# khuongnd6/ViT_torch

Hardware: AMD Instinct MI355X
Metric: images/sec fwd+bwd ViT-B/16 224^2 bs=256/GPU (higher is better)
Workload: dtype bf16; 1 GPU; dino_vitb16 224x224 fwd+CE+bwd+SGD(momentum) step, batch 256/GPU, 10 classes, random-init weights; global_batch=256, residual_stream=bf16, parallelism=dp1, hip_graph=True

## Files before the change

### vit_torch_amd/csrc/layernorm.hip

```cpp
#include <atomic>
#include <initializer_list>
#include <type_traits>
#include "common.h"

namespace {

constexpr int LN_MAXV = 8;

template <int NV, typename TX, typename TY>
__global__ __launch_bounds__(256) void ln_fwd_kernel(const TX* __restrict__ x, int64_t xs,
                                                     const float* __restrict__ gamma,
                                                     const float* __restrict__ beta,
                                                     TY* __restrict__ y, int64_t ys,
                                                     float* __restrict__ mean_out,
                                                     float* __restrict__ rstd_out,
                                                     int64_t M, int D, float eps) {
  const int lane = threadIdx.x & 63, w = threadIdx.x >> 6;
  for (int64_t row = (int64_t)blockIdx.x * 4 + w; row < M; row += (int64_t)gridDim.x * 4) {
  const TX* xr = x + row * xs;
  f32x4 v[NV];
  float s = 0.f;
#pragma unroll
  for (int i = 0; i < NV; ++i) v[i] = load4<TX>(xr + min((i * 64 + lane) * 4, D - 4));
#pragma unroll
  for (int i = 0; i < NV; ++i) {
    const int c = (i * 64 + lane) * 4;
    if (c < D) s += (v[i][0] + v[i][1]) + (v[i][2] + v[i][3]);
  }
  const float mean = wave_sum(s) / (float)D;
  float q = 0.f;
#pragma unroll
  for (int i = 0; i < NV; ++i) {
    const int c = (i * 64 + lane) * 4;
    if (c < D) {
#pragma unroll
      for (int j = 0; j < 4; ++j) { const float d = v[i][j] - mean; q += d * d; }
    }
  }
  const float var = wave_sum(q) / (float)D;
  const float rstd = rsqrtf(var + eps);
  if (lane == 0) {
    if (mean_out) mean_out[row] = mean;
    if (rstd_out) rstd_out[row] = rstd;
  }
  TY* yr = y + row * ys;
#pragma unroll
  for (int i = 0; i < NV; ++i) {
    const int c = (i * 64 + lane) * 4;
    const int cc = min(c, D - 4);
    const f32x4 g = *reinterpret_cast<const f32x4*>(gamma + cc);
    const f32x4 b = *reinterpret_cast<const f32x4*>(beta + cc);
    if (c < D) {
      f32x4 o;
#pragma unroll
      for (int j = 0; j < 4; ++j) o[j] = (v[i][j] - mean) * rstd * g[j] + b[j];
      store4<TY>(yr + c, o);
    }
  }
  }
}

template <int NV, typename TDY, typename TX, typename TG, typename TGB>
__global__ __launch_bounds__(256) void ln_bwd_kernel(const TDY* __restrict__ dy, int64_t dys,
                                                     const TX* __restrict__ x, int64_t xs,
                                                     const float* __restrict__ mean,
                                                     const float* __restrict__ rstd,
                                                     const float* __restrict__ gamma,
                                                     const TG* g_in, TG* g_out, int64_t gstride,
                                                     TGB* __restrict__ gb_out, int64_t gbs,
                                                     float* __restrict__ part, int want_gsum,
                                                     const float* __restrict__ gb_scale,
                                                     const float* __restrict__ gb_rowscale, int64_t rpg,
                                                     int64_t M, int D) {
  extern __shared__ __attribute__((aligned(16))) float red[];
  const int lane = threadIdx.x & 63, w = threadIdx.x >> 6;
  f32x4 gam[NV], dg[NV], db[NV], gs[NV];
#pragma unroll
  for (int i = 0; i < NV; ++i) {
    const int c = (i * 64 + lane) * 4;
    const f32x4 z = {0.f, 0.f, 0.f, 0.f};
    dg[i] = z; db[i] = z; gam[i] = z; gs[i] = z;
    if (c < D) gam[i] = *reinterpret_cast<const f32x4*>(gamma + c);
  }
  const float invD = 1.f / (float)D;
  for (int64_t row = (int64_t)blockIdx.x * 4 + w; row < M; row += (int64_t)gridDim.x * 4) {
    const float mu = mean[row], rs = rstd[row];
    const TDY* dyr = dy + row * dys;
    const TX* xr = x + row * xs;
    f32x4 xh[NV], dv[NV];
    float s1 = 0.f, s2 = 0.f;
#pragma unroll
    for (int i = 0; i < NV; ++i) {
      const int cc = min((i * 64 + lane) * 4, D - 4);
      xh[i] = load4<TX>(xr + cc);
      dv[i] = load4<TDY>(dyr + cc);
    }
#pragma unroll
    for (int i = 0; i < NV; ++i) {
      const int c = (i * 64 + lane) * 4;
      if (c < D) {
        const f32x4 xv = xh[i];
#pragma unroll
        for (int j = 0; j < 4; ++j) {
          xh[i][j] = (xv[j] - mu) * rs;
          dg[i][j] += dv[i][j] * xh[i][j];
          db[i][j] += dv[i][j];
          dv[i][j] *= gam[i][j];
          s1 += dv[i][j];
          s2 += dv[i][j] * xh[i][j];
        }
      }
    }
    const float c1 = wave_sum(s1) * invD, c2 = wave_sum(s2) * invD;
    float rsc = 1.f;
    if (gb_rowscale) rsc = gb_rowscale[(uint32_t)row / (uint32_t)rpg];
    f32x4 gin[NV];
    if (g_in) {
#pragma unroll
      for (int i = 0; i < NV; ++i) gin[i] = load4<TG>(g_in + row * gstride + min((i * 64 + lane) * 4, D - 4));
    }
#pragma unroll
    for (int i = 0; i < NV; ++i) {
      const int c = (i * 64 + lane) * 4;
      if (c < D) {
        f32x4 o;
#pragma unroll
        for (int j = 0; j < 4; ++j) o[j] = rs * (dv[i][j] - c1 - xh[i][j] * c2);
        if (g_in) {
#pragma unroll
          for (int j = 0; j < 4; ++j) o[j] += gin[i][j];
        }
        store4<TG>(g_out + row * gstride + c, o);
        if (gb_scale) {
          const f32x4 sc = *reinterpret_cast<const f32x4*>(gb_scale + c);
#pragma unroll
          for (int j = 0; j < 4; ++j) o[j] *= sc[j];
        }
        if (gb_rowscale) {
#pragma unroll
          for (int j = 0; j < 4; ++j) o[j] *= rsc;
        }
        if (gb_out) store4<TGB>(gb_out + row * gbs + c, o);
#pragma unroll
        for (int j = 0; j < 4; ++j) gs[i][j] += o[j];
      }
    }
  }
  float* prow = part + (int64_t)blockIdx.x * 3 * D;
#pragma unroll 1
  for (int pass = 0; pass < (want_gsum ? 3 : 2); ++pass) {
#pragma unroll
    for (int i = 0; i < NV; ++i) {
      const int c = (i * 64 + lane) * 4;
      if (c < D) *reinterpret_cast<f32x4*>(red + w * D + c) = pass == 0 ? dg[i] : (pass == 1 ? db[i] : gs[i]);
    }
    __syncthreads();
    for (int c = threadIdx.x; c < D; c += 256)
      prow[pass * D + c] = (red[c] + red[D + c]) + (red[2 * D + c] + red[3 * D + c]);
    __syncthreads();
  }
}

template <typename T> __device__ __forceinline__ void load8(const T* p, float (&o)[8]);
template <> __device__ __forceinline__ void load8<float>(const float* p, float (&o)[8]) {
  const f32x4 a = *reinterpret_cast<const f32x4*>(p), b = *reinterpret_cast<const f32x4*>(p + 4);
  o[0] = a[0]; o[1] = a[1]; o[2] = a[2]; o[3] = a[3]; o[4] = b[0]; o[5] = b[1]; o[6] = b[2]; o[7] = b[3];
}
template <> __device__ __forceinline__ void load8<bf16>(const bf16* p, float (&o)[8]) {
  const bf16x8 v = *reinterpret_cast<const bf16x8*>(p);
#pragma unroll
  for (int i = 0; i < 8; ++i) o[i] = (float)v[i];
}
template <typename T> __device__ __forceinline__ void store8(T* p, const float (&v)[8]);
template <> __device__ __forceinline__ void store8<float>(float* p, const float (&v)[8]) {
  *reinterpret_cast<f32x4*>(p) = f32x4{v[0], v[1], v[2], v[3]};
  *reinterpret_cast<f32x4*>(p + 4) = f32x4{v[4], v[5], v[6], v[7]};
}
template <> __device__ __forceinline__ void store8<bf16>(bf16* p, const float (&v)[8]) {
  bf16x8 o;
#pragma unroll
  for (int i = 0; i < 8; ++i) o[i] = (bf16)v[i];
  *reinterpret_cast<bf16x8*>(p) = o;
}
template <int LPR> __device__ __forceinline__ float group_sum(float v) {
#pragma unroll
  for (int o = LPR / 2; o > 0; o >>= 1) v += __shfl_xor(v, o);
  return v;
}

template <int LPR, int NV, typename TX, typename TY>
__global__ __launch_bounds__(256) void ln_fwd8_kernel(const TX* __restrict__ x, int64_t xs, const float* __restrict__ gamma,
                                                      const float* __restrict__ beta, TY* __restrict__ y, int64_t ys,
                                                      float* __restrict__ mean_out, float* __restrict__ rstd_out,
                                                      int64_t M, int D, float eps) {
  constexpr int RPW = 64 / LPR;
  const int lane = threadIdx.x & 63, w = threadIdx.x >> 6;
  const int sub = lane / LPR, l = lane % LPR;
  const int64_t groups = (M + RPW - 1) / RPW;
  const float invD = 1.f / (float)D;
  for (int64_t grp = (int64_t)blockIdx.x * 4 + w; grp < groups; grp += (int64_t)gridDim.x * 4) {
    const int64_t row = grp * RPW + sub;
    const bool live = row < M;
    const TX* xr = x + (live ? row : M - 1) * xs;
    float v[NV][8];
#pragma unroll
    for (int i = 0; i < NV; ++i) load8<TX>(xr + min((i * LPR + l) * 8, D - 8), v[i]);
    float s = 0.f;
#pragma unroll
    for (int i = 0; i < NV; ++i)
      if ((i * LPR + l) * 8 < D) {
#pragma unroll
        for (int j = 0; j < 8; ++j) s += v[i][j];
      }
    const float mean = group_sum<LPR>(s) * invD;
    float q = 0.f;
#pragma unroll
    for (int i = 0; i < NV; ++i)
      if ((i * LPR + l) * 8 < D) {
#pragma unroll
        for (int j = 0; j < 8; ++j) { const float d = v[i][j] - mean; q += d * d; }
      }
    const float rstd = rsqrtf(group_sum<LPR>(q) * invD + eps);
    if (l == 0 && live) {
      if (mean_out) mean_out[row] = mean;
      if (rstd_out) rstd_out[row] = rstd;
    }
    TY* yr = y + row * ys;
#pragma unroll
    for (int i = 0; i < NV; ++i) {
      const int c = (i * LPR + l) * 8;
      float g[8], b[8];
      load8<float>(gamma + min(c, D - 8), g);
      load8<float>(beta + min(c, D - 8), b);
      if (c < D && live) {
        float o[8];
#pragma unroll
        for (int j = 0; j < 8; ++j) o[j] = (v[i][j] - mean) * rstd * g[j] + b[j];
        store8<TY>(yr + c, o);
      }
    }
  }
}

template <int LPR, int NV, typename TDY, typename TX, typename TG, typename TGB>
__global__ __launch_bounds__(256) void ln_bwd8_kernel(const TDY* __restrict__ dy, int64_t dys, const TX* __restrict__ x, int64_t xs,
                                                      const float* __restrict__ mean, const float* __restrict__ rstd,
                                                      const float* __restrict__ gamma, const TG* g_in, TG* g_out, int64_t gstride,
                                                      TGB* __restrict__ gb_out, int64_t gbs, float* __restrict__ part, int want_gsum,
                                                      const float* __restrict__ gb_scale, const float* __restrict__ gb_rowscale,
                                                      int64_t rpg, int64_t M, int D) {
  extern __shared__ __attribute__((aligned(16))) float red[];
  constexpr int RPW = 64 / LPR;
  const int lane = threadIdx.x & 63, w = threadIdx.x >> 6;
  const int sub = lane / LPR, l = lane % LPR;
  float gam[NV][8], dg[NV][8], db[NV][8], gs[NV][8];
#pragma unroll
  for (int i = 0; i < NV; ++i) {
    load8<float>(gamma + min((i * LPR + l) * 8, D - 8), gam[i]);
#pragma unroll
    for (int j = 0; j < 8; ++j) { dg[i][j] = 0.f; db[i][j] = 0.f; gs[i][j] = 0.f; }
  }
  const float invD = 1.f / (float)D;
  const int64_t groups = (M + RPW - 1) / RPW;
  for (int64_t grp = (int64_t)blockIdx.x * 4 + w; grp < groups; grp += (int64_t)gridDim.x * 4) {
    const int64_t row = grp * RPW + sub;
    const bool live = row < M;
    const int64_t r = live ? row : M - 1;
    const float mu = mean[r], rs = rstd[r];
    float xh[NV][8], dv[NV][8], gin[NV][8];
#pragma unroll
    for (int i = 0; i < NV; ++i) {
      const int cc = min((i * LPR + l) * 8, D - 8);
      load8<TX>(x + r * xs + cc, xh[i]);
      load8<TDY>(dy + r * dys + cc, dv[i]);
    }
    if (g_in) {
#pragma unroll
      for (int i = 0; i < NV; ++i) load8<TG>(g_in + r * gstride + min((i * LPR + l) * 8, D - 8), gin[i]);
    }
    float s1 = 0.f, s2 = 0.f;
#pragma unroll
    for (int i = 0; i < NV; ++i)
      if ((i * LPR + l) * 8 < D && live) {
#pragma unroll
        for (int j = 0; j < 8; ++j) {
          xh[i][j] = (xh[i][j] - mu) * rs;
          dg[i][j] += dv[i][j] * xh[i][j];
          db[i][j] += dv[i][j];
          dv[i][j] *= gam[i][j];
          s1 += dv[i][j];
          s2 += dv[i][j] * xh[i][j];
        }
      }
    const float c1 = group_sum<LPR>(s1) * invD, c2 = group_sum<LPR>(s2) * invD;
    float rsc = 1.f;
    if (gb_rowscale) rsc = gb_rowscale[(uint32_t)r / (uint32_t)rpg];
#pragma unroll
    for (int i = 0; i < NV; ++i) {
      const int c = (i * LPR + l) * 8;
      if (c < D && live) {
        float o[8];
#pragma unroll
        for (int j = 0; j < 8; ++j) o[j] = rs * (dv[i][j] - c1 - xh[i][j] * c2);
        if (g_in) {
#pragma unroll
          for (int j = 0; j < 8; ++j) o[j] += gin[i][j];
        }
        store8<TG>(g_out + row * gstride + c, o);
        if (gb_scale) {
          float sc[8];
          load8<float>(gb_scale + c, sc);
#pragma unroll
          for (int j = 0; j < 8; ++j) o[j] *= sc[j];
        }
        if (gb_rowscale) {
#pragma unroll
          for (int j = 0; j < 8; ++j) o[j] *= rsc;
        }
        if (gb_out) store8<TGB>(gb_out + row * gbs + c, o);
#pragma unroll
        for (int j = 0; j < 8; ++j) gs[i][j] += o[j];
      }
    }
  }
  float* prow = part + (int64_t)blockIdx.x * 3 * D;
  const int slot = w * RPW + sub;
#pragma unroll 1
  for (int pass = 0; pass < (want_gsum ? 3 : 2); ++pass) {
#pragma unroll
    for (int i = 0; i < NV; ++i) {
      const int c = (i * LPR + l) * 8;
      float t[8];
#pragma unroll
      for (int j = 0; j < 8; ++j) t[j] = pass == 0 ? dg[i][j] : (pass == 1 ? db[i][j] : gs[i][j]);
      if (c < D) store8<float>(red + slot * D + c, t);
    }
    __syncthreads();
    for (int c = threadIdx.x; c < D; c += 256) {
      float a = 0.f;
#pragma unroll
      for (int t = 0; t < 4 * RPW; ++t) a += red[t * D + c];
      prow[pass * D + c] = a;
    }
    __syncthreads();
  }
}

template <int LPR, int NV, typename T>
__global__ __launch_bounds__(256) void ls_residual_ln_kernel(const float* x, const T* __restrict__ b,
                                                             const float* __restrict__ gamma, const float* __restrict__ lnw,
                                                             const float* __restrict__ lnb, float* y, T* __restrict__ ln,
                                                             float* __restrict__ mean_out, float* __restrict__ rstd_out,
                                                             int64_t M, int D, float eps) {
  constexpr int RPW = 64 / LPR;
  const int lane = threadIdx.x & 63, w = threadIdx.x >> 6;
  const int sub = lane / LPR, l = lane % LPR;
  const int64_t groups = (M + RPW - 1) / RPW;
  const float invD = 1.f / (float)D;
  for (int64_t grp = (int64_t)blockIdx.x * 4 + w; grp < groups; grp += (int64_t)gridDim.x * 4) {
    const int64_t row = grp * RPW + sub;
    const bool live = row < M;
    const int64_t base = row * D;
    float v[NV][8];
    float s = 0.f;
#pragma unroll
    for (int i = 0; i < NV; ++i) {
      const int c = (i * LPR + l) * 8;
      float g[8];
      load8<float>(gamma + min(c, D - 8), g);
      if (live && c < D) {
        float bv[8];
        load8<float>(x + base + c, v[i]);
        load8<T>(b + base + c, bv);
#pragma unroll
        for (int j = 0; j < 8; ++j) {
          v[i][j] = fmaf(g[j], bv[j], v[i][j]);
          s += v[i][j];
        }
        store8<float>(y + base + c, v[i]);
      } else {
#pragma unroll
        for (int j = 0; j < 8; ++j) v[i][j] = 0.f;
      }
    }
    const float mean = group_sum<LPR>(s) * invD;
    float q = 0.f;
#pragma unroll
    for (int i = 0; i < NV; ++i)
      if ((i * LPR + l) * 8 < D) {
#pragma unroll
        for (int j = 0; j < 8; ++j) { const float d = v[i][j] - mean; q += d * d; }
      }
    const float rstd = rsqrtf(group_sum<LPR>(q) * invD + eps);
    if (l == 0 && live) {
      mean_out[row] = mean;
      rstd_out[row] = rstd;
    }
#pragma unroll
    for (int i = 0; i < NV; ++i) {
      const int c = (i * LPR + l) * 8;
      float g[8], bb[8];
      load8<float>(lnw + min(c, D - 8), g);
      load8<float>(lnb + min(c, D - 8), bb);
      if (live && c < D) {
        float o[8];
#pragma unroll
        for (int j = 0; j < 8; ++j) o[j] = (v[i][j] - mean) * rstd * g[j] + bb[j];
        store8<T>(ln + base + c, o);
      }
    }
  }
}

template <int V> using Int = std::integral_constant<int, V>;
template <typename T> struct Type { using type = T; };

struct Ln8Cfg { int lpr, nv; };
inline Ln8Cfg ln8_cfg(int64_t D) {
  if (D <= 128) return {16, 1};
  if (D <= 256) return {16, 2};
  if (D <= 384) return {16, 3};
  if (D <= 512) return {32, 2};
  if (D <= 768) return {32, 3};
  if (D <= 1024) return {64, 2};
  if (D <= 1536) return {64, 3};
  return {64, 4};
}
template <typename F> void with_ln8_cfg(Ln8Cfg c, F&& f) {
  switch (c.lpr * 8 + c.nv) {
    case 16 * 8 + 1: f(Int<16>{}, Int<1>{}); break;
    case 16 * 8 + 2: f(Int<16>{}, Int<2>{}); break;
    case 16 * 8 + 3: f(Int<16>{}, Int<3>{}); break;
    case 32 * 8 + 2: f(Int<32>{}, Int<2>{}); break;
    case 32 * 8 + 3: f(Int<32>{}, Int<3>{}); break;
    case 64 * 8 + 2: f(Int<64>{}, Int<2>{}); break;
    case 64 * 8 + 3: f(Int<64>{}, Int<3>{}); break;
    default: f(Int<64>{}, Int<4>{}); break;
  }
}
static std::atomic<int> g_ln8{1};

inline int ln_nv(int64_t D) { return D <= 512 ? 2 : D <= 768 ? 3 : D <= 1024 ? 4 : LN_MAXV; }
template <typename F> void with_ln_nv(int64_t D, F&& f) {
  switch (ln_nv(D)) {
    case 2: f(Int<2>{}); break;
    case 3: f(Int<3>{}); break;
    case 4: f(Int<4>{}); break;
    default: f(Int<LN_MAXV>{}); break;
  }
}

template <typename F> bool with_fwd_types(int x, int y, F&& f) {
  const Type<float> f32;
  const Type<bf16> b16;
  if (x == VITMI_F32 && y == VITMI_F32) f(f32, f32);
  else if (x == VITMI_F32 && y == VITMI_BF16) f(f32, b16);
  else if (x == VITMI_BF16 && y == VITMI_BF16) f(b16, b16);
  else if (x == VITMI_BF16 && y == VITMI_F32) f(b16, f32);
  else return false;
  return true;
}
template <typename F> bool with_bwd_types(int dy, int x, int g, int gb, F&& f) {
  const Type<float> f32;
  const Type<bf16> b16;
  if (dy == VITMI_F32 && x == VITMI_F32 && g == VITMI_F32 && gb == VITMI_F32) f(f32, f32, f32, f32);
  else if (dy == VITMI_BF16 && x == VITMI_F32 && g == VITMI_F32 && gb == VITMI_BF16) f(b16, f32, f32, b16);
  else if (dy == VITMI_BF16 && x == VITMI_BF16 && g == VITMI_BF16 && gb == VITMI_BF16) f(b16, b16, b16, b16);
  else if (dy == VITMI_F32 && x == VITMI_BF16 && g == VITMI_BF16 && gb == VITMI_F32) f(f32, b16, b16, f32);
  else if (dy == VITMI_F32 && x == VITMI_F32 && g == VITMI_F32 && gb == VITMI_BF16) f(f32, f32, f32, b16);
  else if (dy == VITMI_F32 && x == VITMI_BF16 && g == VITMI_BF16 && gb == VITMI_BF16) f(f32, b16, b16, b16);
  else return false;
  return true;
}

inline unsigned ln_fwd_blocks(int64_t M, int rpw) {
  const int64_t nb = ((M + rpw - 1) / rpw + 3) / 4;
  return (unsigned)(nb < 2048 ? nb : 2048);
}
inline int ln_bwd_blocks(int64_t M, int64_t D) {
  const int nv = ln_nv(D);
  const int64_t cap = nv == 2 ? 1024 : nv <= 4 ? 768 : 512;
  int64_t b = (M + 3) / 4;
  return (int)(b < cap ? b : cap);
}

inline bool ln8_ok(int64_t D, std::initializer_list<int64_t> strides, std::initializer_list<const void*> ptrs) {
  if (!g_ln8 || D % 8 != 0 || D < 8) return false;
  for (int64_t s : strides) if (s % 8 != 0) return false;
  for (const void* p : ptrs) if (p && !is_aligned(p, 16)) return false;
  return true;
}
inline int ln_bwd8_blocks(int64_t M, int64_t D) {
  const Ln8Cfg c = ln8_cfg(D);
  const int64_t groups = (M + 64 / c.lpr - 1) / (64 / c.lpr);
  const int64_t cap = c.nv == 1 ? 1024 : c.nv == 2 ? 768 : c.nv == 3 ? 512 : 256;
  const int64_t b = (groups + 3) / 4;
  return (int)(b < cap ? b : cap);
}

}

extern "C" void vitmi_debug_ln8(int on) { g_ln8 = on != 0; }

static int check_ln_common(const void* x, int x_dtype, int64_t x_stride, int64_t M, int64_t D, const char* who) {
  VITMI_REQUIRE(x && M > 0 && D > 0, VITMI_E_BADARG, "%s: null input or empty shape", who);
  VITMI_REQUIRE(D % 4 == 0 && D <= LN_MAXV * 256, VITMI_E_SHAPE, "%s: D=%lld must be a multiple of 4 and <= %d", who, (long long)D, LN_MAXV * 256);
  VITMI_REQUIRE(x_stride % 4 == 0 && is_aligned(x, 4 * dtype_size(x_dtype)), VITMI_E_ALIGN, "%s: rows must be 4-element aligned", who);
  return 0;
}

extern "C" int vitmi_layernorm_fwd(const void* x, int x_dtype, int64_t x_stride, const float* gamma,
                                   const float* beta, void* y, int y_dtype, int64_t y_stride,
                                   float* mean, float* rstd, int64_t M, int64_t D, float eps,
                                   void* stream_) {
  int rc = check_ln_common(x, x_dtype, x_stride, M, D, "layernorm_fwd");
  if (rc) return rc;
  VITMI_REQUIRE(y && gamma && beta, VITMI_E_BADARG, "layernorm_fwd: null y/gamma/beta");
  VITMI_REQUIRE(y_stride % 4 == 0 && is_aligned(y, 4 * dtype_size(y_dtype)) && is_aligned(gamma, 16) && is_aligned(beta, 16),
                VITMI_E_ALIGN, "layernorm_fwd: y/gamma/beta alignment");
  hipStream_t stream = reinterpret_cast<hipStream_t>(stream_);
  const bool form8 = ln8_ok(D, {x_stride, y_stride}, {x, y, gamma, beta});
  const bool built = with_fwd_types(x_dtype, y_dtype, [&](auto tx, auto ty) {
    using TX = typename decltype(tx)::type;
    using TY = typename decltype(ty)::type;
    auto launch = [&](auto kernel, int rpw) {
      hipLaunchKernelGGL(kernel, dim3(ln_fwd_blocks(M, rpw)), dim3(256), 0, stream, (const TX*)x, x_stride, gamma, beta, (TY*)y,
                         y_stride, mean, rstd, M, (int)D, eps);
    };
    if (form8) with_ln8_cfg(ln8_cfg(D), [&](auto lpr, auto nv) { launch(ln_fwd8_kernel<lpr, nv, TX, TY>, 64 / lpr); });
    else with_ln_nv(D, [&](auto nv) { launch(ln_fwd_kernel<nv, TX, TY>, 1); });
  });
  if (!built) return vitmi_fail(VITMI_E_DTYPE, "layernorm_fwd: dtype combination");
  return vitmi_check_launch(form8 ? "ln_fwd8_kernel" : "ln_fwd_kernel");
}

extern "C" size_t vitmi_layernorm_bwd_workspace(int64_t M, int64_t D) {
  int nb = ln_bwd_blocks(M, D);
  if (D % 8 == 0 && D >= 8) nb = nb > ln_bwd8_blocks(M, D) ? nb : ln_bwd8_blocks(M, D);
  return (size_t)nb * 3 * (size_t)D * sizeof(float);
}

extern "C" int vitmi_layernorm_bwd(const void* dy, int dy_dtype, int64_t dy_stride, const void* x,
                                   int x_dtype, int64_t x_stride, const float* mean,
                                   const float* rstd, const float* gamma, const void* g_in,
                                   void* g_out, int g_dtype, int64_t g_stride, void* gb_out,
                                   int gb_dtype, int64_t gb_stride, float* dgamma, float* dbeta,
                                   float* gsum, const float* gb_scale, const float* gb_rowscale,
                                   int64_t rows_per_group, int64_t M, int64_t D,
                                   void* workspace, size_t workspace_bytes, void* stream_) {
  vitmi_fold_desc fold;
  int rc = vitmi_layernorm_bwd_deferred(dy, dy_dtype, dy_stride, x, x_dtype, x_stride, mean, rstd, gamma, g_in, g_out, g_dtype,
                                        g_stride, gb_out, gb_dtype, gb_stride, dgamma, dbeta, gsum, gb_scale, gb_rowscale,
                                        rows_per_group, M, D, workspace, workspace_bytes, &fold, stream_);
  if (rc) return rc;
  return vitmi_fold_many(&fold, 1, stream_);
}

static void ln_fold_desc(vitmi_fold_desc* f, const float* part, int S, int64_t D, float* dgamma, float* dbeta, float* gsum) {
  f->struct_size = (int64_t)sizeof(vitmi_fold_desc);
  f->part = part; f->S = S; f->nseg = gsum ? 3 : 2; f->N = D; f->ld = 3 * D;
  f->out[0] = dgamma; f->out[1] = dbeta; f->out[2] = gsum;
}

extern "C" int vitmi_layernorm_bwd_deferred(const void* dy, int dy_dtype, int64_t dy_stride, const void* x,
                                            int x_dtype, int64_t x_stride, const float* mean,
                                            const float* rstd, const float* gamma, const void* g_in,
                                            void* g_out, int g_dtype, int64_t g_stride, void* gb_out,
                                            int gb_dtype, int64_t gb_stride, float* dgamma, float* dbeta,
                                            float* gsum, const float* gb_scale, const float* gb_rowscale,
                                            int64_t rows_per_group, int64_t M, int64_t D,
                                            void* workspace, size_t workspace_bytes, vitmi_fold_desc* fold, void* stream_) {
  VITMI_REQUIRE(fold, VITMI_E_BADARG, "layernorm_bwd_deferred: null fold descriptor");
  int rc = check_ln_common(x, x_dtype, x_stride, M, D, "layernorm_bwd");
  if (rc) return rc;
  VITMI_REQUIRE(dy && mean && rstd && gamma && g_out && dgamma && dbeta, VITMI_E_BADARG, "layernorm_bwd: null argument");
  VITMI_REQUIRE(!gb_rowscale || (M < (1ll << 32) && rows_per_group < (1ll << 32)), VITMI_E_SHAPE, "layernorm_bwd: gb_rowscale needs M < 2^32");
  VITMI_REQUIRE(dy_stride % 4 == 0 && g_stride % 4 == 0 && (!gb_out || gb_stride % 4 == 0), VITMI_E_ALIGN, "layernorm_bwd: strides must be multiples of 4");
  VITMI_REQUIRE(is_aligned(dy, 4 * dtype_size(dy_dtype)) && is_aligned(g_out, 4 * dtype_size(g_dtype)) &&
                    (!g_in || is_aligned(g_in, 4 * dtype_size(g_dtype))) &&
                    (!gb_out || is_aligned(gb_out, 4 * dtype_size(gb_dtype))) && is_aligned(gamma, 16) &&
                    (!gb_scale || is_aligned(gb_scale, 16)),
                VITMI_E_ALIGN, "layernorm_bwd: pointer alignment");
  VITMI_REQUIRE(workspace && workspace_bytes >= vitmi_layernorm_bwd_workspace(M, D), VITMI_E_WORKSPACE, "layernorm_bwd: workspace too small");
  VITMI_REQUIRE(is_aligned(workspace, 16), VITMI_E_ALIGN, "layernorm_bwd: workspace alignment");
  hipStream_t stream = reinterpret_cast<hipStream_t>(stream_);
  float* part = reinterpret_cast<float*>(workspace);
  const bool form8 = ln8_ok(D, {dy_stride, x_stride, g_stride, gb_out ? gb_stride : 0}, {dy, x, g_in, g_out, gb_out, gamma, gb_scale});
  const int nb = form8 ? ln_bwd8_blocks(M, D) : ln_bwd_blocks(M, D);
  const size_t lds = (size_t)4 * (form8 ? 64 / ln8_cfg(D).lpr : 1) * D * sizeof(float);
  const int gbd = gb_out ? gb_dtype : dy_dtype;
  const bool built = with_bwd_types(dy_dtype, x_dtype, g_dtype, gbd, [&](auto tdy, auto tx, auto tg, auto tgb) {
    using TDY = typename decltype(tdy)::type;
    using TX = typename decltype(tx)::type;
    using TG = typename decltype(tg)::type;
    using TGB = typename decltype(tgb)::type;
    auto launch = [&](auto kernel) {
      hipLaunchKernelGGL(kernel, dim3(nb), dim3(256), lds, stream, (const TDY*)dy, dy_stride, (const TX*)x, x_stride, mean, rstd,
                         gamma, (const TG*)g_in, (TG*)g_out, g_stride, (TGB*)gb_out, gb_stride, part, gsum ? 1 : 0, gb_scale,
                         gb_rowscale, rows_per_group > 0 ? rows_per_group : 1, M, (int)D);
    };
    if (form8) with_ln8_cfg(ln8_cfg(D), [&](auto lpr, auto nv) { launch(ln_bwd8_kernel<lpr, nv, TDY, TX, TG, TGB>); });
    else with_ln_nv(D, [&](auto nv) { launch(ln_bwd_kernel<nv, TDY, TX, TG, TGB>); });
  });
  if (!built)
    return vitmi_fail(VITMI_E_DTYPE, "layernorm_bwd: dtype combination (dy=%d x=%d g=%d gb=%d)", dy_dtype, x_dtype, g_dtype, gbd);
  rc = vitmi_check_launch(form8 ? "ln_bwd8_kernel" : "ln_bwd_kernel");
  if (rc) return rc;
  ln_fold_desc(fold, part, nb, D, dgamma, dbeta, gsum);
  return 0;
}

static bool lsln_dtype_ok(int dtype) { return dtype == VITMI_BF16 || dtype == VITMI_F32; }
static bool lsln_shape_ok(int64_t M, int64_t D) { return M >= 1 && M < (1ll << 31) && D >= 8 && D % 8 == 0 && D <= LN_MAXV * 256; }

extern "C" int vitmi_ls_residual_ln_supported(int dtype, int64_t M, int64_t D) { return lsln_dtype_ok(dtype) && lsln_shape_ok(M, D); }

extern "C" int vitmi_ls_residual_ln_fwd(const float* x, const void* b, const float* gamma, const float* ln_weight,
                                        const float* ln_bias, float* y, void* l, float* mean, float* rstd, int dtype, int64_t M,
                                        int64_t D, float eps, void* stream) {
  VITMI_REQUIRE(lsln_dtype_ok(dtype), VITMI_E_DTYPE, "ls_residual_ln_fwd: b and l must be bf16 or fp32");
  VITMI_REQUIRE(lsln_shape_ok(M, D), VITMI_E_SHAPE,
                "ls_residual_ln_fwd: M = %lld, D = %lld: M >= 1 (below 2^31), D a multiple of 8 with 8 <= D <= %d", (long long)M,
                (long long)D, LN_MAXV * 256);
  VITMI_REQUIRE(x && b && gamma && ln_weight && ln_bias && y && l && mean && rstd, VITMI_E_BADARG,
                "ls_residual_ln_fwd: null pointer");
  VITMI_REQUIRE(is_aligned(x, 16) && is_aligned(b, 16) && is_aligned(gamma, 16) && is_aligned(ln_weight, 16) &&
                    is_aligned(ln_bias, 16) && is_aligned(y, 16) && is_aligned(l, 16) && is_aligned(mean, 16) &&
                    is_aligned(rstd, 16),
                VITMI_E_ALIGN, "ls_residual_ln_fwd: every pointer must be 16-B aligned");
  VITMI_REQUIRE(eps >= 0.f, VITMI_E_BADARG, "ls_residual_ln_fwd: eps must not be negative");
  hipStream_t s = reinterpret_cast<hipStream_t>(stream);
  auto launch = [&](auto t) {
    using T = typename decltype(t)::type;
    with_ln8_cfg(ln8_cfg(D), [&](auto lpr, auto nv) {
      hipLaunchKernelGGL((ls_residual_ln_kernel<lpr, nv, T>), dim3(ln_fwd_blocks(M, 64 / lpr)), dim3(256), 0, s, x, (const T*)b,
                         gamma, ln_weight, ln_bias, y, (T*)l, mean, rstd, M, (int)D, eps);
    });
  };
  if (dtype == VITMI_BF16) launch(Type<bf16>{});
  else launch(Type<float>{});
  return vitmi_check_launch("ls_residual_ln_kernel");
}

void vitmi_debug_reset_layernorm() {
  g_ln8 = 1;
}
```

Before: 8160 images/sec.

## Prefetch next row group and stage gamma/beta in LDS in LayerNorm forward

The vectorized LayerNorm forward kernel now issues the global loads for the next row group before reducing and normalizing the current one. This software pipelining is meant to hide memory latency in a grid-stride loop. Gamma and beta are staged once per block in shared memory instead of being re-read from global memory for every row. A specialized path for full row groups drops the bounds checks. The cost is higher register pressure from holding two groups of data, plus dynamic LDS use, and the loop makes one extra clamped load past the last group.

```diff
diff --git a/vit_torch_amd/csrc/layernorm.hip b/vit_torch_amd/csrc/layernorm.hip
--- a/vit_torch_amd/csrc/layernorm.hip
+++ b/vit_torch_amd/csrc/layernorm.hip
@@ -6,6 +6,7 @@
 namespace {
 
 constexpr int LN_MAXV = 8;
+template <int V> using Int = std::integral_constant<int, V>;
 
 template <int NV, typename TX, typename TY>
 __global__ __launch_bounds__(256) void ln_fwd_kernel(const TX* __restrict__ x, int64_t xs,
@@ -161,16 +162,26 @@
   }
 }
 
-template <typename T> __device__ __forceinline__ void load8(const T* p, float (&o)[8]);
-template <> __device__ __forceinline__ void load8<float>(const float* p, float (&o)[8]) {
-  const f32x4 a = *reinterpret_cast<const f32x4*>(p), b = *reinterpret_cast<const f32x4*>(p + 4);
-  o[0] = a[0]; o[1] = a[1]; o[2] = a[2]; o[3] = a[3]; o[4] = b[0]; o[5] = b[1]; o[6] = b[2]; o[7] = b[3];
-}
-template <> __device__ __forceinline__ void load8<bf16>(const bf16* p, float (&o)[8]) {
-  const bf16x8 v = *reinterpret_cast<const bf16x8*>(p);
-#pragma unroll
-  for (int i = 0; i < 8; ++i) o[i] = (float)v[i];
-}
+template <typename T> struct Pack8;
+template <> struct Pack8<float> { f32x4 a, b; };
+template <> struct Pack8<bf16> { bf16x8 v; };
+__device__ __forceinline__ Pack8<float> load8p(const float* p) {
+  return {*reinterpret_cast<const f32x4*>(p), *reinterpret_cast<const f32x4*>(p + 4)};
+}
+__device__ __forceinline__ Pack8<bf16> load8p(const bf16* p) { return {*reinterpret_cast<const bf16x8*>(p)}; }
+__device__ __forceinline__ void unpack8(const Pack8<float>& k, float (&o)[8]) {
+  o[0] = k.a[0]; o[1] = k.a[1]; o[2] = k.a[2]; o[3] = k.a[3]; o[4] = k.b[0]; o[5] = k.b[1]; o[6] = k.b[2]; o[7] = k.b[3];
+}
+__device__ __forceinline__ void unpack8(const Pack8<bf16>& k, float (&o)[8]) {
+#pragma unroll
+  for (int i = 0; i < 8; ++i) o[i] = (float)k.v[i];
+}
+template <typename T> __device__ __forceinline__ void load8(const T* p, float (&o)[8]) { unpack8(load8p(p), o); }
+__device__ __forceinline__ void settle8(float (&v)[8]) {
+#pragma unroll
+  for (int j = 0; j < 8; ++j) asm volatile("" : "+v"(v[j]));
+}
+__device__ __forceinline__ void request_fence() { asm volatile("" ::: "memory"); }
 template <typename T> __device__ __forceinline__ void store8(T* p, const float (&v)[8]);
 template <> __device__ __forceinline__ void store8<float>(float* p, const float (&v)[8]) {
   *reinterpret_cast<f32x4*>(p) = f32x4{v[0], v[1], v[2], v[3]};
@@ -193,22 +204,33 @@
                                                       const float* __restrict__ beta, TY* __restrict__ y, int64_t ys,
                                                       float* __restrict__ mean_out, float* __restrict__ rstd_out,
                                                       int64_t M, int D, float eps) {
+  extern __shared__ __attribute__((aligned(16))) float gbs[];
   constexpr int RPW = 64 / LPR;
   const int lane = threadIdx.x & 63, w = threadIdx.x >> 6;
   const int sub = lane / LPR, l = lane % LPR;
   const int64_t groups = (M + RPW - 1) / RPW;
+  const int64_t step = (int64_t)gridDim.x * 4;
   const float invD = 1.f / (float)D;
-  for (int64_t grp = (int64_t)blockIdx.x * 4 + w; grp < groups; grp += (int64_t)gridDim.x * 4) {
+  for (int c = threadIdx.x * 4; c < D; c += 1024) {
+    *reinterpret_cast<f32x4*>(gbs + c) = *reinterpret_cast<const f32x4*>(gamma + c);
+    *reinterpret_cast<f32x4*>(gbs + D + c) = *reinterpret_cast<const f32x4*>(beta + c);
+  }
+  auto request = [&](int64_t g, Pack8<TX> (&p)[NV]) {
+    const TX* xr = x + min(g * RPW + sub, M - 1) * xs;
+#pragma unroll
+    for (int i = 0; i < NV; ++i) p[i] = load8p(xr + min((i * LPR + l) * 8, D - 8));
+  };
+  auto group = [&](auto whole, int64_t grp, float (&v)[NV][8]) {
+    constexpr bool W = decltype(whole)::value;
     const int64_t row = grp * RPW + sub;
-    const bool live = row < M;
-    const TX* xr = x + (live ? row : M - 1) * xs;
-    float v[NV][8];
-#pragma unroll
-    for (int i = 0; i < NV; ++i) load8<TX>(xr + min((i * LPR + l) * 8, D - 8), v[i]);
+    const bool live = W || row < M;
+    Pack8<TX> nxt[NV];
+    request_fence();
+    request(grp + step, nxt);
     float s = 0.f;
 #pragma unroll
     for (int i = 0; i < NV; ++i)
-      if ((i * LPR + l) * 8 < D) {
+      if (W || (i * LPR + l) * 8 < D) {
 #pragma unroll
         for (int j = 0; j < 8; ++j) s += v[i][j];
       }
@@ -216,7 +238,7 @@
     float q = 0.f;
 #pragma unroll
     for (int i = 0; i < NV; ++i)
-      if ((i * LPR + l) * 8 < D) {
+      if (W || (i * LPR + l) * 8 < D) {
 #pragma unroll
         for (int j = 0; j < 8; ++j) { const float d = v[i][j] - mean; q += d * d; }
       }
@@ -230,16 +252,30 @@
     for (int i = 0; i < NV; ++i) {
       const int c = (i * LPR + l) * 8;
       float g[8], b[8];
-      load8<float>(gamma + min(c, D - 8), g);
-      load8<float>(beta + min(c, D - 8), b);
-      if (c < D && live) {
+      load8<float>(gbs + min(c, D - 8), g);
+      load8<float>(gbs + D + min(c, D - 8), b);
+      if (W || (c < D && live)) {
         float o[8];
 #pragma unroll
         for (int j = 0; j < 8; ++j) o[j] = (v[i][j] - mean) * rstd * g[j] + b[j];
         store8<TY>(yr + c, o);
       }
     }
-  }
+#pragma unroll
+    for (int i = 0; i < NV; ++i) { unpack8(nxt[i], v[i]); settle8(v[i]); }
+  };
+  const int64_t whole_groups = NV * LPR * 8 == D ? M / RPW : 0;
+  int64_t grp = (int64_t)blockIdx.x * 4 + w;
+  float v[NV][8];
+  {
+    Pack8<TX> first[NV];
+    request(grp, first);
+    __syncthreads();
+#pragma unroll
+    for (int i = 0; i < NV; ++i) { unpack8(first[i], v[i]); settle8(v[i]); }
+  }
+  for (; grp < whole_groups; grp += step) group(Int<1>{}, grp, v);
+  for (; grp < groups; grp += step) group(Int<0>{}, grp, v);
 }
 
 template <int LPR, int NV, typename TDY, typename TX, typename TG, typename TGB>
@@ -412,7 +448,6 @@
   }
 }
 
-template <int V> using Int = std::integral_constant<int, V>;
 template <typename T> struct Type { using type = T; };
 
 struct Ln8Cfg { int lpr, nv; };
@@ -523,12 +558,12 @@
   const bool built = with_fwd_types(x_dtype, y_dtype, [&](auto tx, auto ty) {
     using TX = typename decltype(tx)::type;
     using TY = typename decltype(ty)::type;
-    auto launch = [&](auto kernel, int rpw) {
-      hipLaunchKernelGGL(kernel, dim3(ln_fwd_blocks(M, rpw)), dim3(256), 0, stream, (const TX*)x, x_stride, gamma, beta, (TY*)y,
+    auto launch = [&](auto kernel, int rpw, size_t lds) {
+      hipLaunchKernelGGL(kernel, dim3(ln_fwd_blocks(M, rpw)), dim3(256), lds, stream, (const TX*)x, x_stride, gamma, beta, (TY*)y,
                          y_stride, mean, rstd, M, (int)D, eps);
     };
-    if (form8) with_ln8_cfg(ln8_cfg(D), [&](auto lpr, auto nv) { launch(ln_fwd8_kernel<lpr, nv, TX, TY>, 64 / lpr); });
-    else with_ln_nv(D, [&](auto nv) { launch(ln_fwd_kernel<nv, TX, TY>, 1); });
+    if (form8) with_ln8_cfg(ln8_cfg(D), [&](auto lpr, auto nv) { launch(ln_fwd8_kernel<lpr, nv, TX, TY>, 64 / lpr, 2 * D * sizeof(float)); });
+    else with_ln_nv(D, [&](auto nv) { launch(ln_fwd_kernel<nv, TX, TY>, 1, 0); });
   });
   if (!built) return vitmi_fail(VITMI_E_DTYPE, "layernorm_fwd: dtype combination");
   return vitmi_check_launch(form8 ? "ln_fwd8_kernel" : "ln_fwd_kernel");
```

Result: no change. 8184 images/sec, median of 4 (+0.3%).
